# microsoft/CryptoNets

Hardware: AMD Instinct MI355X
Metric: encrypted images/sec (CryptoNets-MNIST, N=8192) (higher is better)
Workload: dtype u64

## Files before the change

### cryptonets_amd/csrc/cn_k_rr.hip.h

```cpp
#pragma once
#include "cn_dev_common.hip.h"

template <int L, class AR, bool inverse>
__global__ void __launch_bounds__(NttPlan<L>::NT) k_ntt_rr(uint64_t *data, const DevConsts *__restrict__ C, uint32_t base_off, uint32_t nmod) {
    typedef typename AR::T T;
    extern __shared__ __align__(16) unsigned char smem[];
    T *s = reinterpret_cast<T *>(smem);
    constexpr uint32_t n = 1u << L;
    constexpr int SA = NttPlan<L>::SA;
    const uint32_t tid = threadIdx.x, mod = base_off + blockIdx.x % nmod;
    const ArCtx<AR> A(C, mod);
    uint64_t *x = data + (size_t)blockIdx.x * n;
    T v[16];
    if (!inverse) {
#pragma unroll
        for (int r = 0; r < 16; r++) v[r] = A.load(x[pass_index<L, SA, 0>(tid, r)]);
        ntt_forward_regs<AR, L>(v, s, A.fw, A.m, tid);
#pragma unroll
        for (int r = 0; r < 16; r += 2) {
            ulonglong2 o; o.x = A.canon(v[r]); o.y = A.canon(v[r + 1]);
            *reinterpret_cast<ulonglong2 *>(x + tail_index<L>(tid, r)) = o;
        }
    } else {
#pragma unroll
        for (int r = 0; r < 16; r += 2) {
            ulonglong2 i2 = *reinterpret_cast<const ulonglong2 *>(x + tail_index<L>(tid, r));
            v[r] = A.load(i2.x); v[r + 1] = A.load(i2.y);
        }
        ntt_inverse_regs<AR, L>(v, s, A.iv, A.m, tid);
#pragma unroll
        for (int r = 0; r < 16; r++) x[pass_index<L, SA, 0>(tid, r)] = A.scaled(v[r]);
    }
}
template <int L, class AR>
__global__ void __launch_bounds__(NttPlan<L>::NT) k_lift_ntt(const uint64_t *__restrict__ pt, uint32_t pitch, uint64_t *__restrict__ lifted, const DevConsts *__restrict__ C) {
    typedef typename AR::T T;
    extern __shared__ __align__(16) unsigned char smem[];
    T *s = reinterpret_cast<T *>(smem);
    constexpr uint32_t n = 1u << L;
    constexpr int SA = NttPlan<L>::SA;
    const uint32_t tid = threadIdx.x, k = C->k, j = blockIdx.x % k, pi = blockIdx.x / k;
    const ArCtx<AR> A(C, j);
    const uint64_t *x = pt + (size_t)pi * pitch * n, th = C->t_half, inc = C->lift_inc[j];
    T v[16];
#pragma unroll
    for (int r = 0; r < 16; r++) { const uint64_t m = x[pass_index<L, SA, 0>(tid, r)]; v[r] = A.load(m >= th ? m + inc : m); }
    ntt_forward_regs<AR, L>(v, s, A.fw, A.m, tid);
    uint64_t *o = lifted + (size_t)blockIdx.x * n;
#pragma unroll
    for (int r = 0; r < 16; r += 2) {
        ulonglong2 w; w.x = A.canon(v[r]); w.y = A.canon(v[r + 1]);
        *reinterpret_cast<ulonglong2 *>(o + tail_index<L>(tid, r)) = w;
    }
}
template <int L, class AR, bool PTN = false>
__global__ void __launch_bounds__(NttPlan<L>::NT) k_mul_plain_bcast(const uint64_t *__restrict__ pt, uint32_t pitch, const uint64_t *__restrict__ ctn, uint64_t *__restrict__ out,
                                                                    const DevConsts *__restrict__ C, uint32_t polys, uint32_t next_elt, uint64_t *__restrict__ next_out) {
    typedef typename AR::T T;
    extern __shared__ __align__(16) unsigned char smem[];
    T *s = reinterpret_cast<T *>(smem);
    constexpr uint32_t n = 1u << L;
    constexpr int SA = NttPlan<L>::SA;
    const uint32_t tid = threadIdx.x, k = C->k, j = blockIdx.x % k, cp = blockIdx.x / k, row = cp / polys, p = cp % polys;
    const ArCtx<AR> A(C, j);
    const TensorOps<AR> ops(C, j);
    const uint64_t *w = ctn + ((size_t)p * k + j) * n;
    T v[16];
    uint32_t tm = tid;
    if constexpr (PTN) {
        const uint64_t *x = pt + (((size_t)row * pitch) * k + j) * n;
#pragma unroll
        for (int r = 0; r < 16; r += 2) {
            const ulonglong2 m = *reinterpret_cast<const ulonglong2 *>(x + tail_index<L>(tm, r));
            v[r] = A.load(m.x); v[r + 1] = A.load(m.y);
        }
    } else {
        const uint64_t *x = pt + (size_t)row * pitch * n, th = C->t_half, inc = C->lift_inc[j];
#pragma unroll
        for (int r = 0; r < 16; r++) { const uint64_t m = x[pass_index<L, SA, 0>(tid, r)]; v[r] = A.load(m >= th ? m + inc : m); }
        ntt_forward_regs<AR, L>(v, s, A.fw, A.m, tid);
        asm volatile("" : "+v"(tm));
    }
#pragma unroll
    for (int r = 0; r < 16; r += 2) {
        const ulonglong2 y = *reinterpret_cast<const ulonglong2 *>(w + tail_index<L>(tm, r));
        if constexpr (std::is_same<T, double>::value) {
            v[r] = ops.mul(v[r], A.load(y.x), A); v[r + 1] = ops.mul(v[r + 1], A.load(y.y), A);
        } else if constexpr (PTN) {
            v[r] = ops.mul(v[r], y.x, A); v[r + 1] = ops.mul(v[r + 1], y.y, A);
        } else {
            v[r] = ops.mul(A.canon(v[r]), y.x, A); v[r + 1] = ops.mul(A.canon(v[r + 1]), y.y, A);
        }
    }
    if (!PTN && !ntt_tail_local<L>()) __syncthreads();
    uint32_t ti = tid;
    asm volatile("" : "+v"(ti));
    ntt_inverse_regs<AR, L>(v, s, A.iv, A.m, ti);
    uint64_t *o = out + ((size_t)cp * k + j) * n;
    const bool chain = next_elt && p == 1;
    uint64_t *win = reinterpret_cast<uint64_t *>(smem);
    if (chain) __syncthreads();
#pragma unroll
    for (int r = 0; r < 16; r++) {
        const uint32_t e = pass_index<L, SA, 0>(ti, r);
        const uint64_t val = A.scaled(v[r]);
        o[e] = val;
        if (chain) { const uint32_t pos = (e * next_elt) & (2 * n - 1); win[pos & (n - 1)] = (pos >> L) ? negmod(val, C->q[j].q) : val; }
    }
    if (chain) {
        __syncthreads();
        uint64_t *no = next_out + ((size_t)row * k + j) * n;
#pragma unroll
        for (int r = 0; r < 16; r++) no[ti + NttPlan<L>::NT * (uint32_t)r] = win[ti + NttPlan<L>::NT * (uint32_t)r];
    }
}
template <int L, class AR>
__global__ void __launch_bounds__(NttPlan<L>::NT) k_mul_plain_fused(const uint64_t *src, size_t src_stride, const uint64_t *__restrict__ ptn, uint32_t pstride,
                                                                    uint64_t *out, const DevConsts *__restrict__ C, uint32_t polys) {
    typedef typename AR::T T;
    extern __shared__ __align__(16) unsigned char smem[];
    T *s = reinterpret_cast<T *>(smem);
    constexpr uint32_t n = 1u << L;
    constexpr int SA = NttPlan<L>::SA;
    const uint32_t tid = threadIdx.x, k = C->k, j = blockIdx.x % k, cp = blockIdx.x / k, ct = cp / polys, p = cp % polys;
    const ArCtx<AR> A(C, j);
    const TensorOps<AR> ops(C, j);
    const uint64_t *x = src + (size_t)ct * src_stride + ((size_t)p * k + j) * n;
    const uint64_t *w = ptn + ((size_t)ct * pstride * k + j) * n;
    T v[16];
#pragma unroll
    for (int r = 0; r < 16; r++) v[r] = A.load(x[pass_index<L, SA, 0>(tid, r)]);
    ntt_forward_regs<AR, L>(v, s, A.fw, A.m, tid);
    uint32_t tm = tid;
    asm volatile("" : "+v"(tm));
#pragma unroll
    for (int r = 0; r < 16; r += 2) {
        const ulonglong2 y = *reinterpret_cast<const ulonglong2 *>(w + tail_index<L>(tm, r));
        if constexpr (std::is_same<T, double>::value) {
            v[r] = ops.mul(v[r], A.load(y.x), A); v[r + 1] = ops.mul(v[r + 1], A.load(y.y), A);
        } else {
            v[r] = ops.mul(A.canon(v[r]), y.x, A); v[r + 1] = ops.mul(A.canon(v[r + 1]), y.y, A);
        }
    }
    if (!ntt_tail_local<L>()) __syncthreads();
    uint32_t ti = tid;
    asm volatile("" : "+v"(ti));
    ntt_inverse_regs<AR, L>(v, s, A.iv, A.m, ti);
    uint64_t *o = out + ((size_t)cp * k + j) * n;
#pragma unroll
    for (int r = 0; r < 16; r++) o[pass_index<L, SA, 0>(ti, r)] = A.scaled(v[r]);
}

template <int L, class AR>
__global__ void __launch_bounds__(NttPlan<L>::NT) k_intt_tensor(const uint64_t *__restrict__ A_, const uint64_t *__restrict__ B_, uint64_t *__restrict__ D,
                                                                const DevConsts *__restrict__ C, uint32_t base_off, uint32_t Lm, uint32_t lazy) {
    typedef typename AR::T T;
    extern __shared__ __align__(16) unsigned char smem[];
    T *s = reinterpret_cast<T *>(smem);
    constexpr uint32_t n = 1u << L;
    constexpr int SA = NttPlan<L>::SA;
    const uint32_t tid = threadIdx.x;
    const uint32_t l = blockIdx.x % Lm, p = (blockIdx.x / Lm) % 3, ct = blockIdx.x / (3 * Lm), mod = base_off + l;
    const ArCtx<AR> A(C, mod);
    const TensorOps<AR> ops(C, mod);
    const size_t Ln = (size_t)Lm * n;
    const uint64_t *a0 = A_ + (size_t)ct * 2 * Ln + (size_t)l * n, *a1 = a0 + Ln;
    const uint64_t *b0 = B_ + (size_t)ct * 2 * Ln + (size_t)l * n, *b1 = b0 + Ln;
    T v[16];
#pragma unroll
    for (int r = 0; r < 16; r += 2) {
        const uint32_t pos = tail_index<L>(tid, r);
        if (p == 0) {
            const ulonglong2 x = *reinterpret_cast<const ulonglong2 *>(a0 + pos), y = *reinterpret_cast<const ulonglong2 *>(b0 + pos);
            v[r] = ops.mul(A.load(x.x), A.load(y.x), A); v[r + 1] = ops.mul(A.load(x.y), A.load(y.y), A);
        } else if (p == 2) {
            const ulonglong2 x = *reinterpret_cast<const ulonglong2 *>(a1 + pos), y = *reinterpret_cast<const ulonglong2 *>(b1 + pos);
            v[r] = ops.mul(A.load(x.x), A.load(y.x), A); v[r + 1] = ops.mul(A.load(x.y), A.load(y.y), A);
        } else {
            const ulonglong2 x0 = *reinterpret_cast<const ulonglong2 *>(a0 + pos), y1 = *reinterpret_cast<const ulonglong2 *>(b1 + pos);
            const ulonglong2 x1 = *reinterpret_cast<const ulonglong2 *>(a1 + pos), y0 = *reinterpret_cast<const ulonglong2 *>(b0 + pos);
            v[r] = ops.add(ops.mul(A.load(x0.x), A.load(y1.x), A), ops.mul(A.load(x1.x), A.load(y0.x), A));
            v[r + 1] = ops.add(ops.mul(A.load(x0.y), A.load(y1.y), A), ops.mul(A.load(x1.y), A.load(y0.y), A));
        }
    }
    ntt_inverse_regs<AR, L>(v, s, A.iv, A.m, tid);
    uint64_t *o = D + ((size_t)ct * 3 + p) * Ln + (size_t)l * n;
    if constexpr (std::is_same<T, double>::value) {
        if (lazy) {
#pragma unroll
            for (int r = 0; r < 16; r++) o[pass_index<L, SA, 0>(tid, r)] = lazy_word(v[r]);
            return;
        }
    }
#pragma unroll
    for (int r = 0; r < 16; r++) o[pass_index<L, SA, 0>(tid, r)] = A.scaled(v[r]);
}

struct NttOut01 {};
template <int L, class AR, bool PLDS = false, class... NX_>
__global__ void __launch_bounds__(NttPlan<L>::NT, PLDS ? 2 : 4) k_square_fused(const uint64_t *__restrict__ A_, size_t a_stride, const uint64_t *const *__restrict__ a_tab,
                                                                    uint64_t *__restrict__ D, const DevConsts *__restrict__ C, uint32_t base_off, uint32_t Lm) {
    typedef typename AR::T T;
    constexpr bool NX = sizeof...(NX_) != 0;
    static_assert(std::is_same<T, double>::value, "FP64 policies only");
    extern __shared__ __align__(16) unsigned char smem[];
    T *s = reinterpret_cast<T *>(smem);
    constexpr uint32_t n = 1u << L;
    constexpr int SA = NttPlan<L>::SA;
    const uint32_t tid = threadIdx.x;
    const uint32_t l = blockIdx.x % Lm, ct = blockIdx.x / Lm, mod = base_off + l;
    const ArCtx<AR> A(C, mod);
    const size_t Ln = (size_t)Lm * n;
    const NTT_GLOBAL uint64_t *a0 = (const NTT_GLOBAL uint64_t *)(a_tab ? a_tab[ct] : A_ + (size_t)ct * a_stride) + (size_t)l * n, *a1 = a0 + Ln;
    uint64_t *d0 = D + (size_t)ct * 3 * Ln + (size_t)l * n, *d1 = d0 + Ln, *d2 = d1 + Ln;
    struct alignas(16) P2 { T a, b; };
    P2 *pk = reinterpret_cast<P2 *>(s + ntt_lds_words(n)) + tid;
#pragma unroll 1
    for (int step = 0; step < 3; step++) {
        uint32_t tl = tid;
        asm volatile("" : "+v"(tl));
        T v[16];
        if (step < 2) {
            const NTT_GLOBAL uint64_t *x = step ? a1 : a0;
#pragma unroll
            for (int r = 0; r < 16; r++) v[r] = A.load(x[pass_index<L, SA, 0>(tl, r)]);
            ntt_forward_regs<AR, L, true>(v, s, A.fw, A.m, tl);
            AR::renorm(v, A.m);
            if constexpr (PLDS) {
                if (step == 0) {
#pragma unroll
                    for (int r = 0; r < 16; r += 2) pk[(r >> 1) * NttPlan<L>::NT] = P2{v[r], v[r + 1]};
#pragma unroll
                    for (int r = 0; r < 16; r++) v[r] = AR::mulmod(v[r], v[r], A.m);
                } else {
#pragma unroll
                    for (int r = 0; r < 16; r += 2) {
                        const P2 w = pk[(r >> 1) * NttPlan<L>::NT];
                        pk[(r >> 1) * NttPlan<L>::NT] = P2{v[r], v[r + 1]};
                        v[r] = AR::mulmod(__dadd_rn(w.a, w.a), v[r], A.m); v[r + 1] = AR::mulmod(__dadd_rn(w.b, w.b), v[r + 1], A.m);
                    }
                }
            } else {
            uint64_t *park = step ? d2 : d1;
#pragma unroll
            for (int r = 0; r < 16; r += 2) {
                ulonglong2 w; w.x = (uint64_t)__double_as_longlong(v[r]); w.y = (uint64_t)__double_as_longlong(v[r + 1]);
                *reinterpret_cast<ulonglong2 *>(park + tail_index<L>(tl, r)) = w;
            }
            if (step == 0) {
#pragma unroll
                for (int r = 0; r < 16; r++) v[r] = AR::mulmod(v[r], v[r], A.m);
            } else {
#pragma unroll
                for (int r = 0; r < 16; r += 2) {
                    const ulonglong2 w = *reinterpret_cast<const ulonglong2 *>(d1 + tail_index<L>(tl, r));
                    const T wa = __longlong_as_double((long long)w.x), wb = __longlong_as_double((long long)w.y);
                    v[r] = AR::mulmod(__dadd_rn(wa, wa), v[r], A.m); v[r + 1] = AR::mulmod(__dadd_rn(wb, wb), v[r + 1], A.m);
                }
            }
            }
            if (!ntt_tail_local<L>()) __syncthreads();
        } else {
#pragma unroll
            for (int r = 0; r < 16; r += 2) {
                T wa, wb;
                if constexpr (PLDS) { const P2 w = pk[(r >> 1) * NttPlan<L>::NT]; wa = w.a; wb = w.b; }
                else {
                    const ulonglong2 w = *reinterpret_cast<const ulonglong2 *>(d2 + tail_index<L>(tl, r));
                    wa = __longlong_as_double((long long)w.x); wb = __longlong_as_double((long long)w.y);
                }
                v[r] = AR::mulmod(wa, wa, A.m); v[r + 1] = AR::mulmod(wb, wb, A.m);
            }
            __syncthreads();
        }
        if constexpr (NX) {
            static_assert(!NX || PLDS, "NTT-form d0, d1: the LDS-parked form only");
            if (step < 2) {
                uint64_t *on = step ? d1 : d0;
#pragma unroll
                for (int r = 0; r < 16; r += 2) {
                    ulonglong2 w; w.x = A.canon(v[r]); w.y = A.canon(v[r + 1]);
                    *reinterpret_cast<ulonglong2 *>(on + tail_index<L>(tl, r)) = w;
                }
                continue;
            }
        }
        uint32_t ti = tid;
        asm volatile("" : "+v"(ti));
        ntt_inverse_regs<AR, L>(v, s, A.iv, A.m, ti);
        uint64_t *o = step == 0 ? d0 : (step == 1 ? d1 : d2);
        uint32_t to = tid;
        asm volatile("" : "+v"(to));
#pragma unroll
        for (int r = 0; r < 16; r++) o[pass_index<L, SA, 0>(to, r)] = lazy_word(v[r]);
    }
}
template <class AR> struct LdsTwiddles;
template <int RN> struct LdsTwiddles<ArF64T<RN>> { typedef ArF64LdsT<RN> type; };
template <int L, class AR, class... NX_>
__global__ void __launch_bounds__(NttPlan<L>::NT, 2) k_square_pipe(const uint64_t *__restrict__ A_, size_t a_stride, const uint64_t *const *__restrict__ a_tab,
                                                                    uint64_t *__restrict__ D, const DevConsts *__restrict__ C, uint32_t base_off, uint32_t Lm, uint32_t cnt) {
    typedef typename AR::T T;
    constexpr bool NX = sizeof...(NX_) != 0;
    static_assert(std::is_same<T, double>::value && L <= 13, "FP64 policies, N <= 8192");
    extern __shared__ __align__(16) unsigned char smem[];
    T *s = reinterpret_cast<T *>(smem);
    constexpr uint32_t n = 1u << L;
    constexpr int SA = NttPlan<L>::SA;
    const uint32_t tid = threadIdx.x;
    const uint32_t G = gridDim.x / Lm, l = blockIdx.x % Lm, w0 = blockIdx.x / Lm, mod = base_off + l;
    const ArCtx<AR> A(C, mod);
    const size_t Ln = (size_t)Lm * n;
    typedef ArPassA<AR> FW;
    typename FW::Tw fwt;
    static_cast<typename AR::Tw &>(fwt) = A.fw;
    ntt_load_pass_a<SA>(fwt, A.fw.w);
    typedef typename LdsTwiddles<AR>::type IV;
    typename IV::Tw ivt;
    {
        double *tws = reinterpret_cast<double *>(smem) + ntt_lds_words(n);
        stage_table(tws, A.iv.w, n, tid, NttPlan<L>::NT);
        ivt.w = (const __attribute__((address_space(3))) double *)tws;
        __syncthreads();
    }
    auto operand = [&](uint32_t ct) { return (const NTT_GLOBAL uint64_t *)(a_tab ? a_tab[ct] : A_ + (size_t)ct * a_stride) + (size_t)l * n; };
    uint64_t nxt[16];
    {
        const NTT_GLOBAL uint64_t *x = operand(w0);
#pragma unroll
        for (int r = 0; r < 16; r++) nxt[r] = x[pass_index<L, SA, 0>(tid, r)];
    }
    for (uint32_t ct = w0; ct < cnt; ct += G) {
        uint64_t *d0 = D + (size_t)ct * 3 * Ln + (size_t)l * n;
        T P[16];
#pragma unroll 1
        for (int step = 0; step < 3; step++) {
            uint32_t tl = tid;
            asm volatile("" : "+v"(tl));
            T v[16];
            if (step < 2) {
#pragma unroll
                for (int r = 0; r < 16; r++) v[r] = A.load(nxt[r]);
                ntt_forward_regs<FW, L, true>(v, s, fwt, A.m, tl);
                AR::renorm(v, A.m);
                {
                    const uint32_t nct = step ? (ct + G < cnt ? ct + G : ct) : ct;
                    const NTT_GLOBAL uint64_t *x = operand(nct) + (step ? 0 : Ln);
                    uint32_t tp = tid;
                    asm volatile("" : "+v"(tp));
#pragma unroll
                    for (int r = 0; r < 16; r++) nxt[r] = x[pass_index<L, SA, 0>(tp, r)];
                }
                if (step == 0) {
#pragma unroll
                    for (int r = 0; r < 16; r++) { P[r] = v[r]; v[r] = AR::mulmod(v[r], v[r], A.m); }
                } else {
#pragma unroll
                    for (int r = 0; r < 16; r++) { const T a0 = P[r]; P[r] = v[r]; v[r] = AR::mulmod(__dadd_rn(a0, a0), v[r], A.m); }
                }
                if (!ntt_tail_local<L>()) __syncthreads();
            } else {
#pragma unroll
                for (int r = 0; r < 16; r++) v[r] = AR::mulmod(P[r], P[r], A.m);
                __syncthreads();
            }
            if constexpr (NX) {
                if (step < 2) {
                    uint64_t *on = d0 + (size_t)step * Ln;
#pragma unroll
                    for (int r = 0; r < 16; r += 2) {
                        ulonglong2 w; w.x = A.canon(v[r]); w.y = A.canon(v[r + 1]);
                        *reinterpret_cast<ulonglong2 *>(on + tail_index<L>(tl, r)) = w;
                    }
                    continue;
                }
            }
            uint32_t ti = tid;
            asm volatile("" : "+v"(ti));
            ntt_inverse_regs<IV, L>(v, s, ivt, A.m, ti);
            uint64_t *o = d0 + (size_t)step * Ln;
            uint32_t to = tid;
            asm volatile("" : "+v"(to));
#pragma unroll
            for (int r = 0; r < 16; r++) o[pass_index<L, SA, 0>(to, r)] = lazy_word(v[r]);
        }
    }
}
template <class AR> struct EncTail {
    typedef typename AR::T T;
    const ArCtx<AR> &A; const DevConsts *C; uint32_t j; uint64_t q, t_half; double dlt, rtq;
    NTT_DEV EncTail(const ArCtx<AR> &A_, const DevConsts *C_, uint32_t j_, uint64_t q_) : A(A_), C(C_), j(j_), q(q_), t_half(C_->t_half), dlt((double)C_->delta[j_]), rtq((double)C_->rtq[j_]) {}
    NTT_DEV uint64_t word(T v, int32_t ns, bool has_m, uint64_t mw) const {
        if constexpr (std::is_same<T, double>::value) {
            double x = __dadd_rn(AR::mulmod(v, A.ni, A.m), (double)ns);
            if (has_m) {
                double y = AR::mulmod(AR::from_u64(mw), dlt, A.m);
                if (mw >= t_half) y = __dadd_rn(y, rtq);
                x = __dadd_rn(x, y);
            }
            return AR::to_u64(x, A.m);
        } else {
            uint64_t val = A.scaled(v);
            val = addmod(val, ns >= 0 ? (uint64_t)ns : q - (uint64_t)(-ns), q);
            if (has_m) val = addmod(val, scale_plain(C, mw, j), q);
            return val;
        }
    }
};
template <int L, class AR>
__global__ void __launch_bounds__(NttPlan<L>::NT) k_encrypt_tail(const uint64_t *__restrict__ u, const uint64_t *__restrict__ pk, const uint64_t *__restrict__ pt,
                                                                 uint32_t pt_stride_words, uint64_t *__restrict__ out, const DevConsts *__restrict__ C,
                                                                 const int8_t *__restrict__ noise, const EncTab *__restrict__ tab) {
    typedef typename AR::T T;
    extern __shared__ __align__(16) unsigned char smem[];
    T *s = reinterpret_cast<T *>(smem);
    constexpr uint32_t n = 1u << L;
    constexpr int SA = NttPlan<L>::SA;
    const uint32_t k = C->k, tid = threadIdx.x, j = blockIdx.x % k, p = (blockIdx.x / k) & 1, ct = blockIdx.x / (2 * k);
    const ArCtx<AR> A(C, j);
    const TensorOps<AR> ops(C, j);
    const uint64_t *uu = u + ((size_t)ct * k + j) * n, *pp = pk + ((size_t)p * k + j) * n;
    T v[16];
#pragma unroll
    for (int r = 0; r < 16; r += 2) {
        const uint32_t pos = tail_index<L>(tid, r);
        const ulonglong2 x = *reinterpret_cast<const ulonglong2 *>(uu + pos), y = *reinterpret_cast<const ulonglong2 *>(pp + pos);
        v[r] = ops.mul(A.load(x.x), A.load(y.x), A); v[r + 1] = ops.mul(A.load(x.y), A.load(y.y), A);
    }
    ntt_inverse_regs<AR, L>(v, s, A.iv, A.m, tid);
    NTT_GLOBAL uint64_t *o = (tab ? tab[ct].out : (NTT_GLOBAL uint64_t *)out + (size_t)ct * 2 * k * n) + ((size_t)p * k + j) * n;
    const NTT_GLOBAL uint64_t *m = tab ? tab[ct].pt : (pt ? (const NTT_GLOBAL uint64_t *)pt + (size_t)ct * pt_stride_words : nullptr);
    const int8_t *ee = noise + ((size_t)ct * 2 + p) * n;
    const uint64_t q = C->q[j].q;
    const EncTail<AR> tail(A, C, j, q);
    const bool has_m = p == 0 && m;
#pragma unroll
    for (int r = 0; r < 16; r++) {
        const uint32_t e = pass_index<L, SA, 0>(tid, r);
        o[e] = tail.word(v[r], ee[e], has_m, has_m ? m[e] : 0);
    }
}

template <int L, class AR>
__global__ void __launch_bounds__(NttPlan<L>::NT) k_encrypt_fused(const int8_t *__restrict__ us, const uint64_t *__restrict__ pk, const uint64_t *__restrict__ pt,
                                                                  uint32_t pt_stride_words, uint64_t *__restrict__ out, const DevConsts *__restrict__ C,
                                                                  const int8_t *__restrict__ noise, const EncTab *__restrict__ tab) {
    typedef typename AR::T T;
    extern __shared__ __align__(16) unsigned char smem[];
    T *s = reinterpret_cast<T *>(smem);
    constexpr uint32_t n = 1u << L;
    constexpr int SA = NttPlan<L>::SA;
    const uint32_t k = C->k, tid = threadIdx.x, j = blockIdx.x % k, ct = blockIdx.x / k;
    const ArCtx<AR> A(C, j);
    const TensorOps<AR> ops(C, j);
    const uint64_t q = C->q[j].q;
    T U[16];
    {
        const int8_t *uu = us + (size_t)ct * n;
#pragma unroll
        for (int r = 0; r < 16; r++) { const int32_t v = uu[pass_index<L, SA, 0>(tid, r)]; U[r] = A.load(v >= 0 ? (uint64_t)v : q - (uint64_t)(-v)); }
        ntt_forward_regs<AR, L>(U, s, A.fw, A.m, tid);
        if constexpr (std::is_same<T, double>::value) AR::renorm(U, A.m);
        else {
#pragma unroll
            for (int r = 0; r < 16; r++) U[r] = A.canon(U[r]);
        }
    }
    NTT_GLOBAL uint64_t *obase = tab ? tab[ct].out : (NTT_GLOBAL uint64_t *)out + (size_t)ct * 2 * k * n;
    const NTT_GLOBAL uint64_t *m = tab ? tab[ct].pt : (pt ? (const NTT_GLOBAL uint64_t *)pt + (size_t)ct * pt_stride_words : nullptr);
#pragma unroll 1
    for (int p = 0; p < 2; p++) {
        uint32_t tl = tid;
        asm volatile("" : "+v"(tl));
        const uint64_t *pp = pk + ((size_t)p * k + j) * n;
        T v[16];
#pragma unroll
        for (int r = 0; r < 16; r += 2) {
            const ulonglong2 y = *reinterpret_cast<const ulonglong2 *>(pp + tail_index<L>(tl, r));
            v[r] = ops.mul(U[r], A.load(y.x), A); v[r + 1] = ops.mul(U[r + 1], A.load(y.y), A);
        }
        if (p || !ntt_tail_local<L>()) __syncthreads();
        ntt_inverse_regs<AR, L>(v, s, A.iv, A.m, tl);
        NTT_GLOBAL uint64_t *o = obase + ((size_t)p * k + j) * n;
        const int8_t *ee = noise + ((size_t)ct * 2 + p) * n;
        const EncTail<AR> tail(A, C, j, q);
        const bool has_m = p == 0 && m;
#pragma unroll
        for (int r = 0; r < 16; r++) {
            const uint32_t e = pass_index<L, SA, 0>(tl, r);
            o[e] = tail.word(v[r], ee[e], has_m, has_m ? m[e] : 0);
        }
    }
}

template <int L, class AR>
__global__ void __launch_bounds__(NttPlan<L>::NT, 4) k_encrypt_split(const int8_t *__restrict__ us, const uint64_t *__restrict__ pk, const uint64_t *__restrict__ pt,
                                                                     uint32_t pt_stride_words, uint64_t *__restrict__ out, const DevConsts *__restrict__ C,
                                                                     const int8_t *__restrict__ noise, const EncTab *__restrict__ tab) {
    typedef typename AR::T T;
    extern __shared__ __align__(16) unsigned char smem[];
    T *s = reinterpret_cast<T *>(smem);
    constexpr uint32_t n = 1u << L;
    constexpr int SA = NttPlan<L>::SA;
    const uint32_t k = C->k, tid = threadIdx.x, j = blockIdx.x % k, p = (blockIdx.x / k) & 1, ct = blockIdx.x / (2 * k);
    const ArCtx<AR> A(C, j);
    const TensorOps<AR> ops(C, j);
    const uint64_t q = C->q[j].q;
    T v[16];
    {
        const int8_t *uu = us + (size_t)ct * n;
#pragma unroll
        for (int r = 0; r < 16; r++) { const int32_t x = uu[pass_index<L, SA, 0>(tid, r)]; v[r] = A.load(x >= 0 ? (uint64_t)x : q - (uint64_t)(-x)); }
        ntt_forward_regs<AR, L>(v, s, A.fw, A.m, tid);
        if constexpr (std::is_same<T, double>::value) AR::renorm(v, A.m);
        else {
#pragma unroll
            for (int r = 0; r < 16; r++) v[r] = A.canon(v[r]);
        }
    }
    const uint64_t *pp = pk + ((size_t)p * k + j) * n;
#pragma unroll
    for (int r = 0; r < 16; r += 2) {
        const ulonglong2 y = *reinterpret_cast<const ulonglong2 *>(pp + tail_index<L>(tid, r));
        v[r] = ops.mul(v[r], A.load(y.x), A); v[r + 1] = ops.mul(v[r + 1], A.load(y.y), A);
    }
    if (!ntt_tail_local<L>()) __syncthreads();
    ntt_inverse_regs<AR, L>(v, s, A.iv, A.m, tid);
    NTT_GLOBAL uint64_t *o = (tab ? tab[ct].out : (NTT_GLOBAL uint64_t *)out + (size_t)ct * 2 * k * n) + ((size_t)p * k + j) * n;
    const NTT_GLOBAL uint64_t *m = tab ? tab[ct].pt : (pt ? (const NTT_GLOBAL uint64_t *)pt + (size_t)ct * pt_stride_words : nullptr);
    const int8_t *ee = noise + ((size_t)ct * 2 + p) * n;
    const EncTail<AR> tail(A, C, j, q);
    const bool has_m = p == 0 && m;
#pragma unroll
    for (int r = 0; r < 16; r++) {
        const uint32_t e = pass_index<L, SA, 0>(tid, r);
        o[e] = tail.word(v[r], ee[e], has_m, has_m ? m[e] : 0);
    }
}

template <int L, class AR>
__global__ void __launch_bounds__(NttPlan<L>::NT, 4) k_encrypt_fold(const int8_t *__restrict__ us, const uint64_t *__restrict__ pk, const DevConsts *__restrict__ C,
                                                                    const int8_t *__restrict__ noise, const FoldOut *__restrict__ fout, const FoldTerm *__restrict__ terms) {
    typedef typename AR::T T;
    static_assert(std::is_same<T, double>::value, "FP64 policies only");
    extern __shared__ __align__(16) unsigned char smem[];
    T *s = reinterpret_cast<T *>(smem);
    constexpr uint32_t n = 1u << L;
    constexpr int SA = NttPlan<L>::SA;
    const uint32_t k = C->k, tid = threadIdx.x, j = blockIdx.x % k, p = (blockIdx.x / k) & 1, ct = blockIdx.x / (2 * k);
    const ArCtx<AR> A(C, j);
    const TensorOps<AR> ops(C, j);
    const FoldOut fo = fout[ct];
    const FoldTerm *tt = terms + fo.first;
    auto accumulate = [&](T (&X)[16], const int8_t *base, size_t pitch, size_t off) {
        uint32_t t = 0;
#pragma unroll 1
        for (; t + 3 <= fo.count; t += 3) {
            int8_t b[3][16];
#pragma unroll
            for (int c = 0; c < 3; c++) {
                const int8_t *pp = base + (size_t)tt[t + c].enc * pitch + off;
#pragma unroll
                for (int r = 0; r < 16; r++) b[c][r] = pp[pass_index<L, SA, 0>(tid, r)];
            }
#pragma unroll
            for (int c = 0; c < 3; c++) {
                const double w = tt[t + c].w;
#pragma unroll
                for (int r = 0; r < 16; r++) X[r] = __fma_rn(w, (double)(int32_t)b[c][r], X[r]);
            }
        }
#pragma unroll 1
        for (; t < fo.count; t++) {
            const double w = tt[t].w;
            const int8_t *pp = base + (size_t)tt[t].enc * pitch + off;
#pragma unroll
            for (int r = 0; r < 16; r++) X[r] = __fma_rn(w, (double)(int32_t)pp[pass_index<L, SA, 0>(tid, r)], X[r]);
        }
    };
    T v[16];
#pragma unroll
    for (int r = 0; r < 16; r++) v[r] = 0.0;
    accumulate(v, us, n, 0);
    AR::renorm(v, A.m);
    ntt_forward_regs<AR, L>(v, s, A.fw, A.m, tid);
    AR::renorm(v, A.m);
    const uint64_t *pp = pk + ((size_t)p * k + j) * n;
#pragma unroll
    for (int r = 0; r < 16; r += 2) {
        const ulonglong2 y = *reinterpret_cast<const ulonglong2 *>(pp + tail_index<L>(tid, r));
        v[r] = ops.mul(v[r], A.load(y.x), A); v[r + 1] = ops.mul(v[r + 1], A.load(y.y), A);
    }
    if (!ntt_tail_local<L>()) __syncthreads();
    ntt_inverse_regs<AR, L>(v, s, A.iv, A.m, tid);
    T E[16];
#pragma unroll
    for (int r = 0; r < 16; r++) E[r] = 0.0;
    accumulate(E, noise, (size_t)2 * n, (size_t)p * n);
    NTT_GLOBAL uint64_t *o = (NTT_GLOBAL uint64_t *)fo.out + ((size_t)p * k + j) * n;
#pragma unroll
    for (int r = 0; r < 16; r++) {
        const uint32_t e = pass_index<L, SA, 0>(tid, r);
        const double x = __dadd_rn(__dadd_rn(AR::mulmod(v[r], A.ni, A.m), AR::center(E[r], A.m)), AR::from_u64(o[e]));
        o[e] = AR::to_u64(x, A.m);
    }
}
```

### cryptonets_amd/csrc/cn_ntt_core.hip.h

```cpp
#pragma once
#include <hip/hip_runtime.h>
#include <stdint.h>

#define NTT_DEV __device__ __forceinline__
#define NTT_GLOBAL __attribute__((address_space(1)))
#ifndef NTT_STAGE_FENCE
#define NTT_STAGE_FENCE 0
#endif
#ifndef NTT_FWD_RECENTRE_ALL
#define NTT_FWD_RECENTRE_ALL 0
#endif
#ifndef NTT_TAIL_LOCAL
#define NTT_TAIL_LOCAL 1
#endif

NTT_DEV uint32_t lds_pos(uint32_t e) { return e + 2u * (e >> 5); }
__host__ __device__ constexpr inline uint32_t ntt_lds_words(uint32_t n) { return n + 2u * (n >> 5); }

NTT_DEV uint64_t ntt_mulshoup(uint64_t y, uint64_t w, uint64_t ws, uint64_t q) { return y * w - __umul64hi(ws, y) * q; }

struct ArU64 {
    typedef uint64_t T;
    struct Mod { uint64_t q, q2; };
    struct Tw { const NTT_GLOBAL uint64_t *w; const NTT_GLOBAL uint64_t *ws; };
    static NTT_DEV void fwd(T &X, T &Y, const Tw &t, uint32_t ti, const Mod &m) {
        const uint64_t W = t.w[ti], Ws = t.ws[ti];
        uint64_t x = X - ((X >= m.q2) ? m.q2 : 0);
        uint64_t p = ntt_mulshoup(Y, W, Ws, m.q);
        X = x + p;
        Y = x + m.q2 - p;
    }
    static NTT_DEV void inv(T &U, T &V, const Tw &t, uint32_t ti, const Mod &m) {
        const uint64_t W = t.w[ti], Ws = t.ws[ti];
        uint64_t s = U + V, d = U + m.q2 - V;
        U = s - ((s >= m.q2) ? m.q2 : 0);
        V = ntt_mulshoup(d, W, Ws, m.q);
    }
    template <int SITE> static NTT_DEV void renorm_at(T (&)[16], const Mod &) {}
    static NTT_DEV void renorm(T (&)[16], const Mod &) {}
};

enum { RS_FWD_B = 0, RS_INV_START = 1, RS_INV_C = 2, RS_INV_B = 3, RS_INV_A = 4, RS_FWD_C = 5, RS_FWD_TAIL = 6 };

template <int RN> struct ArF64T {
    typedef double T;
    struct Mod { double q, qinv; };
    struct Tw { const NTT_GLOBAL double *w; };
    static NTT_DEV double mulmod(double y, double w, const Mod &m) {
        const double p = __dmul_rn(y, w);
        const double e = __fma_rn(y, w, -p);
        const double h = __builtin_rint(__dmul_rn(p, m.qinv));
        return __dadd_rn(__fma_rn(-h, m.q, p), e);
    }
    static NTT_DEV double center(double x, const Mod &m) {
        return __fma_rn(-__builtin_rint(__dmul_rn(x, m.qinv)), m.q, x);
    }
    static NTT_DEV void fwd(T &X, T &Y, const Tw &t, uint32_t ti, const Mod &m) {
        const double p = mulmod(Y, t.w[ti], m);
        Y = __dadd_rn(X, -p);
        X = __dadd_rn(X, p);
    }
    static NTT_DEV void inv(T &U, T &V, const Tw &t, uint32_t ti, const Mod &m) {
        const double s = __dadd_rn(U, V), d = __dadd_rn(U, -V);
        U = s;
        V = mulmod(d, t.w[ti], m);
    }
    static NTT_DEV void renorm(T (&x)[16], const Mod &m) {
#pragma unroll
        for (int r = 0; r < 16; r++) x[r] = center(x[r], m);
    }
    template <int SITE> static NTT_DEV void renorm_at(T (&x)[16], const Mod &m) {
        if (SITE == RS_FWD_B || SITE == RS_FWD_TAIL) { if (NTT_FWD_RECENTRE_ALL && RN == 1) renorm(x, m); }
        else if (RN == 1 || SITE == RS_INV_START || SITE == RS_INV_B || SITE == RS_INV_A) renorm(x, m);
    }
    static NTT_DEV uint64_t to_u64(double x, const Mod &m) {
        double r = center(x, m);
        r = r < 0.0 ? __dadd_rn(r, m.q) : r;
        return (uint64_t)__double_as_longlong(__dadd_rn(r, 4503599627370496.0)) & 0x000FFFFFFFFFFFFFull;
    }
    static NTT_DEV double from_u64(uint64_t v) {
        return __dadd_rn(__longlong_as_double((long long)(v | 0x4330000000000000ull)), -4503599627370496.0);
    }
};
typedef ArF64T<1> ArF64;
typedef ArF64T<0> ArF64L;
template <int RN> struct ArF64LdsT : ArF64T<RN> {
    typedef typename ArF64T<RN>::T T;
    typedef typename ArF64T<RN>::Mod Mod;
    struct Tw { const __attribute__((address_space(3))) double *w; };
    static NTT_DEV void fwd(T &X, T &Y, const Tw &t, uint32_t ti, const Mod &m) {
        const double p = ArF64T<RN>::mulmod(Y, t.w[ti], m);
        Y = __dadd_rn(X, -p);
        X = __dadd_rn(X, p);
    }
    static NTT_DEV void inv(T &U, T &V, const Tw &t, uint32_t ti, const Mod &m) {
        const double s = __dadd_rn(U, V), d = __dadd_rn(U, -V);
        U = s;
        V = ArF64T<RN>::mulmod(d, t.w[ti], m);
    }
};

NTT_DEV double ntt_uniform(double v) {
    const uint64_t b = (uint64_t)__double_as_longlong(v);
    const uint32_t lo = __builtin_amdgcn_readfirstlane((uint32_t)b), hi = __builtin_amdgcn_readfirstlane((uint32_t)(b >> 32));
    return __longlong_as_double((long long)(((uint64_t)hi << 32) | lo));
}
template <class BASE> struct ArPassA : BASE {
    typedef typename BASE::T T;
    typedef typename BASE::Mod Mod;
    struct Tw : BASE::Tw { double wa[16]; };
    static constexpr bool passA = true;
    static NTT_DEV void fwdA(T &X, T &Y, const Tw &t, int ti, const Mod &m) {
        const double p = BASE::mulmod(Y, t.wa[ti], m);
        Y = __dadd_rn(X, -p);
        X = __dadd_rn(X, p);
    }
    static NTT_DEV void invA(T &U, T &V, const Tw &t, int ti, const Mod &m) {
        const double s = __dadd_rn(U, V), d = __dadd_rn(U, -V);
        U = s;
        V = BASE::mulmod(d, t.wa[ti], m);
    }
};
template <class AR, class = void> struct HasPassA { static constexpr bool value = false; };
template <class AR> struct HasPassA<AR, decltype((void)AR::passA)> { static constexpr bool value = true; };
template <int SA, class TW> NTT_DEV void ntt_load_pass_a(TW &t, const NTT_GLOBAL double *table) {
#pragma unroll
    for (int i = 1; i < (1 << SA); i++) t.wa[i] = ntt_uniform(table[i]);
}

template <int L> struct NttPlan {
    static constexpr int D = (L == 14) ? 2 : 1;
    static constexpr int SA = L - 8 - D;
    static constexpr int NT = 1 << (L - 4);
    static_assert(SA >= 1 && SA <= 4, "unsupported transform size");
};

template <int L, int S, int S0> NTT_DEV uint32_t pass_index(uint32_t tid, int r) {
    constexpr int NT = 1 << (L - 4), LO = L - S0 - S;
    const uint32_t G = (uint32_t)(r >> S) * NT + tid, mid = r & ((1 << S) - 1);
    const uint32_t lo = G & ((1u << LO) - 1), hi = G >> LO;
    return (hi << (L - S0)) | (mid << LO) | lo;
}
template <int L, int S, int S0> NTT_DEV uint32_t pass_hi(uint32_t tid, int g) {
    constexpr int NT = 1 << (L - 4), LO = L - S0 - S;
    return ((uint32_t)g * NT + tid) >> LO;
}

template <class AR, int L, int S, int S0> NTT_DEV void fwd_stages(typename AR::T (&x)[16], const typename AR::Tw &tw, const typename AR::Mod &m, uint32_t tid) {
#pragma unroll
    for (int u = 0; u < S; u++) {
        if (NTT_STAGE_FENCE) __builtin_amdgcn_sched_barrier(0);
        const int half = 1 << (S - 1 - u);
#pragma unroll
        for (int g = 0; g < (16 >> S); g++) {
            const uint32_t hi = S0 == 0 ? 0u : pass_hi<L, S, S0>(tid, g);
#pragma unroll
            for (int blk = 0; blk < (1 << u); blk++) {
                const uint32_t ti = (1u << (S0 + u)) + ((hi << u) | (uint32_t)blk);
#pragma unroll
                for (int j = 0; j < half; j++) {
                    const int a = (g << S) + blk * 2 * half + j;
                    if constexpr (S0 == 0 && HasPassA<AR>::value) AR::fwdA(x[a], x[a + half], tw, (1 << u) + blk, m);
                    else AR::fwd(x[a], x[a + half], tw, ti, m);
                }
            }
        }
    }
}
template <class AR, int L, int S, int S0> NTT_DEV void inv_stages(typename AR::T (&x)[16], const typename AR::Tw &tw, const typename AR::Mod &m, uint32_t tid) {
#pragma unroll
    for (int u = S - 1; u >= 0; u--) {
        if (NTT_STAGE_FENCE) __builtin_amdgcn_sched_barrier(0);
        const int half = 1 << (S - 1 - u);
#pragma unroll
        for (int g = 0; g < (16 >> S); g++) {
            const uint32_t hi = S0 == 0 ? 0u : pass_hi<L, S, S0>(tid, g);
#pragma unroll
            for (int blk = 0; blk < (1 << u); blk++) {
                const uint32_t ti = (1u << (S0 + u)) + ((hi << u) | (uint32_t)blk);
#pragma unroll
                for (int j = 0; j < half; j++) {
                    const int a = (g << S) + blk * 2 * half + j;
                    if constexpr (S0 == 0 && HasPassA<AR>::value) AR::invA(x[a], x[a + half], tw, (1 << u) + blk, m);
                    else AR::inv(x[a], x[a + half], tw, ti, m);
                }
            }
        }
    }
}
template <class T> struct NttBaseOffset { static constexpr bool value = false; };
template <> struct NttBaseOffset<double> { static constexpr bool value = true; };
template <class T, int L, int S, int S0> NTT_DEV void lds_put(const T (&x)[16], T *s, uint32_t tid) {
    if constexpr (NttBaseOffset<T>::value) {
        T *b = s + lds_pos(pass_index<L, S, S0>(tid, 0));
#pragma unroll
        for (int r = 0; r < 16; r++) b[lds_pos(pass_index<L, S, S0>(0u, r))] = x[r];
    } else {
#pragma unroll
        for (int r = 0; r < 16; r++) s[lds_pos(pass_index<L, S, S0>(tid, r))] = x[r];
    }
}
template <class T, int L, int S, int S0> NTT_DEV void lds_get(T (&x)[16], const T *s, uint32_t tid) {
    if constexpr (NttBaseOffset<T>::value) {
        const T *b = s + lds_pos(pass_index<L, S, S0>(tid, 0));
#pragma unroll
        for (int r = 0; r < 16; r++) x[r] = b[lds_pos(pass_index<L, S, S0>(0u, r))];
    } else {
#pragma unroll
        for (int r = 0; r < 16; r++) x[r] = s[lds_pos(pass_index<L, S, S0>(tid, r))];
    }
}
template <int L> constexpr bool ntt_tail_local() { return NTT_TAIL_LOCAL && NttPlan<L>::D == 1; }
template <int L> NTT_DEV uint32_t tail_index(uint32_t tid, int r) {
    constexpr int D = NttPlan<L>::D, NT = NttPlan<L>::NT;
    if (ntt_tail_local<L>())
        return ((tid >> 5) << 9) + (((tid & 31u) + 32u * (uint32_t)(r >> 1)) << 1) + (uint32_t)(r & 1);
    return ((tid + (uint32_t)NT * (uint32_t)(r >> D)) << D) + (uint32_t)(r & ((1 << D) - 1));
}
template <class T, int L> NTT_DEV void lds_put_tail(const T (&x)[16], T *s, uint32_t tid) {
#pragma unroll
    for (int r = 0; r < 16; r += 2) {
        struct alignas(16) P2 { T a, b; } v{x[r], x[r + 1]};
        *reinterpret_cast<P2 *>(s + lds_pos(tail_index<L>(tid, r))) = v;
    }
}
template <class T, int L> NTT_DEV void lds_get_tail(T (&x)[16], const T *s, uint32_t tid) {
#pragma unroll
    for (int r = 0; r < 16; r += 2) {
        struct alignas(16) P2 { T a, b; };
        const P2 v = *reinterpret_cast<const P2 *>(s + lds_pos(tail_index<L>(tid, r)));
        x[r] = v.a; x[r + 1] = v.b;
    }
}
template <class AR, int L> NTT_DEV void fwd_tail(typename AR::T (&x)[16], const typename AR::Tw &tw, const typename AR::Mod &m, uint32_t tid) {
    constexpr int D = NttPlan<L>::D, NT = NttPlan<L>::NT;
    if (D == 2) {
#pragma unroll
        for (int g = 0; g < 4; g++) {
            const uint32_t c = tid + (uint32_t)NT * g, t0 = (1u << (L - 2)) + c;
            AR::fwd(x[4 * g], x[4 * g + 2], tw, t0, m);
            AR::fwd(x[4 * g + 1], x[4 * g + 3], tw, t0, m);
        }
    }
#pragma unroll
    for (int p = 0; p < 8; p++) {
        const uint32_t pair = tail_index<L>(tid, 2 * p) >> 1, ti = (1u << (L - 1)) + pair;
        AR::fwd(x[2 * p], x[2 * p + 1], tw, ti, m);
    }
}
template <class AR, int L> NTT_DEV void inv_tail(typename AR::T (&x)[16], const typename AR::Tw &tw, const typename AR::Mod &m, uint32_t tid) {
    constexpr int D = NttPlan<L>::D, NT = NttPlan<L>::NT;
#pragma unroll
    for (int p = 0; p < 8; p++) {
        const uint32_t pair = tail_index<L>(tid, 2 * p) >> 1, ti = (1u << (L - 1)) + pair;
        AR::inv(x[2 * p], x[2 * p + 1], tw, ti, m);
    }
    if (D == 2) {
#pragma unroll
        for (int g = 0; g < 4; g++) {
            const uint32_t c = tid + (uint32_t)NT * g, t0 = (1u << (L - 2)) + c;
            AR::inv(x[4 * g], x[4 * g + 2], tw, t0, m);
            AR::inv(x[4 * g + 1], x[4 * g + 3], tw, t0, m);
        }
    }
}

NTT_DEV void ntt_wave_sync() {
    __builtin_amdgcn_fence(__ATOMIC_RELEASE, "wavefront");
    __builtin_amdgcn_wave_barrier();
    __builtin_amdgcn_fence(__ATOMIC_ACQUIRE, "wavefront");
}
template <class AR, int L, bool PRE = false> NTT_DEV void ntt_forward_regs(typename AR::T (&x)[16], typename AR::T *s, const typename AR::Tw &tw, const typename AR::Mod &m, uint32_t tid) {
    typedef typename AR::T T;
    constexpr int SA = NttPlan<L>::SA;
    fwd_stages<AR, L, SA, 0>(x, tw, m, tid);
    if (PRE) __syncthreads();
    lds_put<T, L, SA, 0>(x, s, tid);
    __syncthreads();
    lds_get<T, L, 4, SA>(x, s, tid);
    AR::template renorm_at<RS_FWD_B>(x, m);
    fwd_stages<AR, L, 4, SA>(x, tw, m, tid);
    lds_put<T, L, 4, SA>(x, s, tid);
    ntt_wave_sync();
    lds_get<T, L, 4, SA + 4>(x, s, tid);
    AR::template renorm_at<RS_FWD_C>(x, m);
    fwd_stages<AR, L, 4, SA + 4>(x, tw, m, tid);
    lds_put<T, L, 4, SA + 4>(x, s, tid);
    if (ntt_tail_local<L>()) ntt_wave_sync(); else __syncthreads();
    lds_get_tail<T, L>(x, s, tid);
    AR::template renorm_at<RS_FWD_TAIL>(x, m);
    fwd_tail<AR, L>(x, tw, m, tid);
}
template <class AR, int L, bool PRE, class HK> NTT_DEV void ntt_forward_regs_hooked(typename AR::T (&x)[16], typename AR::T *s, const typename AR::Tw &tw, const typename AR::Mod &m,
                                                                                     uint32_t tid, HK &hk) {
    typedef typename AR::T T;
    constexpr int SA = NttPlan<L>::SA;
    hk.template at<0>();
    fwd_stages<AR, L, SA, 0>(x, tw, m, tid);
    hk.template at<1>();
    if (PRE) __syncthreads();
    lds_put<T, L, SA, 0>(x, s, tid);
    __syncthreads();
    lds_get<T, L, 4, SA>(x, s, tid);
    AR::template renorm_at<RS_FWD_B>(x, m);
    fwd_stages<AR, L, 4, SA>(x, tw, m, tid);
    hk.template at<2>();
    lds_put<T, L, 4, SA>(x, s, tid);
    ntt_wave_sync();
    lds_get<T, L, 4, SA + 4>(x, s, tid);
    AR::template renorm_at<RS_FWD_C>(x, m);
    fwd_stages<AR, L, 4, SA + 4>(x, tw, m, tid);
    hk.template at<3>();
    lds_put<T, L, 4, SA + 4>(x, s, tid);
    if (ntt_tail_local<L>()) ntt_wave_sync(); else __syncthreads();
    lds_get_tail<T, L>(x, s, tid);
    AR::template renorm_at<RS_FWD_TAIL>(x, m);
    fwd_tail<AR, L>(x, tw, m, tid);
}
template <class AR, int L> NTT_DEV void ntt_inverse_regs(typename AR::T (&x)[16], typename AR::T *s, const typename AR::Tw &tw, const typename AR::Mod &m, uint32_t tid) {
    typedef typename AR::T T;
    constexpr int SA = NttPlan<L>::SA;
    AR::template renorm_at<RS_INV_START>(x, m);
    inv_tail<AR, L>(x, tw, m, tid);
    lds_put_tail<T, L>(x, s, tid);
    if (ntt_tail_local<L>()) ntt_wave_sync(); else __syncthreads();
    lds_get<T, L, 4, SA + 4>(x, s, tid);
    AR::template renorm_at<RS_INV_C>(x, m);
    inv_stages<AR, L, 4, SA + 4>(x, tw, m, tid);
    lds_put<T, L, 4, SA + 4>(x, s, tid);
    ntt_wave_sync();
    lds_get<T, L, 4, SA>(x, s, tid);
    AR::template renorm_at<RS_INV_B>(x, m);
    inv_stages<AR, L, 4, SA>(x, tw, m, tid);
    lds_put<T, L, 4, SA>(x, s, tid);
    __syncthreads();
    lds_get<T, L, SA, 0>(x, s, tid);
    AR::template renorm_at<RS_INV_A>(x, m);
    inv_stages<AR, L, SA, 0>(x, tw, m, tid);
}
```

Before: 1.322 million.

## Stage forward twiddles in LDS and keep last-stage twiddles in registers

In the fused square pipeline, the forward twiddle table now also comes from LDS: the first half of each table is staged (forward and inverse share the LDS region). The final-stage twiddles for each thread's eight butterfly pairs are preloaded into registers once per block, for both forward and inverse transforms. This removes repeated global twiddle fetches in the tail stages across the per-ciphertext loop. The cost is extra VGPR pressure (16 doubles), which could hurt occupancy under the 2-blocks launch bound, and the kernel is restricted to D=1 sizes.

```diff
diff --git a/cryptonets_amd/csrc/cn_k_rr.hip.h b/cryptonets_amd/csrc/cn_k_rr.hip.h
--- a/cryptonets_amd/csrc/cn_k_rr.hip.h
+++ b/cryptonets_amd/csrc/cn_k_rr.hip.h
@@ -311,16 +311,19 @@
     const uint32_t G = gridDim.x / Lm, l = blockIdx.x % Lm, w0 = blockIdx.x / Lm, mod = base_off + l;
     const ArCtx<AR> A(C, mod);
     const size_t Ln = (size_t)Lm * n;
-    typedef ArPassA<AR> FW;
+    typedef ArTailRegs<ArPassA<typename LdsTwiddles<AR>::type>> FW;
+    typedef ArTailRegs<typename LdsTwiddles<AR>::type> IV;
     typename FW::Tw fwt;
-    static_cast<typename AR::Tw &>(fwt) = A.fw;
-    ntt_load_pass_a<SA>(fwt, A.fw.w);
-    typedef typename LdsTwiddles<AR>::type IV;
     typename IV::Tw ivt;
     {
+        typedef const __attribute__((address_space(3))) double *LP;
         double *tws = reinterpret_cast<double *>(smem) + ntt_lds_words(n);
-        stage_table(tws, A.iv.w, n, tid, NttPlan<L>::NT);
-        ivt.w = (const __attribute__((address_space(3))) double *)tws;
+        stage_table(tws, A.fw.w, n / 2, tid, NttPlan<L>::NT);
+        stage_table(tws + n / 2, A.iv.w, n / 2, tid, NttPlan<L>::NT);
+        fwt.w = (LP)tws; ivt.w = (LP)(tws + n / 2);
+        ntt_load_pass_a<SA>(fwt, A.fw.w);
+        ntt_load_tail<L>(fwt, A.fw.w, tid);
+        ntt_load_tail<L>(ivt, A.iv.w, tid);
         __syncthreads();
     }
     auto operand = [&](uint32_t ct) { return (const NTT_GLOBAL uint64_t *)(a_tab ? a_tab[ct] : A_ + (size_t)ct * a_stride) + (size_t)l * n; };
diff --git a/cryptonets_amd/csrc/cn_ntt_core.hip.h b/cryptonets_amd/csrc/cn_ntt_core.hip.h
--- a/cryptonets_amd/csrc/cn_ntt_core.hip.h
+++ b/cryptonets_amd/csrc/cn_ntt_core.hip.h
@@ -128,6 +128,25 @@
     for (int i = 1; i < (1 << SA); i++) t.wa[i] = ntt_uniform(table[i]);
 }
 
+template <class BASE> struct ArTailRegs : BASE {
+    typedef typename BASE::T T;
+    typedef typename BASE::Mod Mod;
+    struct Tw : BASE::Tw { double wt[8]; };
+    static constexpr bool tailRegs = true;
+    static NTT_DEV void fwdT(T &X, T &Y, const Tw &t, int p, const Mod &m) {
+        const double r = BASE::mulmod(Y, t.wt[p], m);
+        Y = __dadd_rn(X, -r);
+        X = __dadd_rn(X, r);
+    }
+    static NTT_DEV void invT(T &U, T &V, const Tw &t, int p, const Mod &m) {
+        const double s = __dadd_rn(U, V), d = __dadd_rn(U, -V);
+        U = s;
+        V = BASE::mulmod(d, t.wt[p], m);
+    }
+};
+template <class AR, class = void> struct HasTailRegs { static constexpr bool value = false; };
+template <class AR> struct HasTailRegs<AR, decltype((void)AR::tailRegs)> { static constexpr bool value = true; };
+
 template <int L> struct NttPlan {
     static constexpr int D = (L == 14) ? 2 : 1;
     static constexpr int SA = L - 8 - D;
@@ -232,8 +251,19 @@
         x[r] = v.a; x[r + 1] = v.b;
     }
 }
+template <int L, class TW> NTT_DEV void ntt_load_tail(TW &t, const NTT_GLOBAL double *table, uint32_t tid) {
+    static_assert(NttPlan<L>::D == 1, "one root per register pair: D = 1");
+#pragma unroll
+    for (int p = 0; p < 8; p++) t.wt[p] = table[(1u << (L - 1)) + (tail_index<L>(tid, 2 * p) >> 1)];
+}
 template <class AR, int L> NTT_DEV void fwd_tail(typename AR::T (&x)[16], const typename AR::Tw &tw, const typename AR::Mod &m, uint32_t tid) {
     constexpr int D = NttPlan<L>::D, NT = NttPlan<L>::NT;
+    if constexpr (HasTailRegs<AR>::value) {
+        static_assert(D == 1, "ArTailRegs: D = 1");
+#pragma unroll
+        for (int p = 0; p < 8; p++) AR::fwdT(x[2 * p], x[2 * p + 1], tw, p, m);
+        return;
+    }
     if (D == 2) {
 #pragma unroll
         for (int g = 0; g < 4; g++) {
@@ -250,6 +280,12 @@
 }
 template <class AR, int L> NTT_DEV void inv_tail(typename AR::T (&x)[16], const typename AR::Tw &tw, const typename AR::Mod &m, uint32_t tid) {
     constexpr int D = NttPlan<L>::D, NT = NttPlan<L>::NT;
+    if constexpr (HasTailRegs<AR>::value) {
+        static_assert(D == 1, "ArTailRegs: D = 1");
+#pragma unroll
+        for (int p = 0; p < 8; p++) AR::invT(x[2 * p], x[2 * p + 1], tw, p, m);
+        return;
+    }
 #pragma unroll
     for (int p = 0; p < 8; p++) {
         const uint32_t pair = tail_index<L>(tid, 2 * p) >> 1, ti = (1u << (L - 1)) + pair;
```

Result: faster. 1.340 million (median of 6 runs) (+1.3%).
